# dojo-sim/Dojo.jl

Measured on NVIDIA H100. Metric: env-steps/sec (forward step!), higher is better.
Workload: dtype f64

## Files before the change

### dojo.jl_b200/csrc/dojo_b200.cu

```cuda
#include <cuda_runtime.h>

#include <algorithm>
#include <climits>
#include <cstdio>
#include <cstdlib>
#include <cstring>
#include <string>
#include <vector>

#include "../../include/dojo_b200.h"
#include "dojo_step_kernel.cuh"
#include "dojo_kin.cuh"
#include "dojo_kinjac.cuh"
#include "dojo_envs.cuh"
#include "dojo_storage.cuh"

using namespace dj;

extern "C" __attribute__((visibility("hidden"))) const void* dojo_cm_step_kernel(int grad);
static const void* step_kernel_fn(bool any_contact, bool grad, bool plan_smem, bool small = false) {
  if (any_contact) return dojo_cm_step_kernel(grad ? 1 : 0);
  if (plan_smem && !getenv("DOJO_B200_GENERIC_PLAN")) {
    if (!grad && small) return (const void*)dojo_step_kernel<false, true, false, true>;
    return grad ? (const void*)dojo_step_kernel<true, true> : (const void*)dojo_step_kernel<false, true>;
// ... 290 lines not shown

  Plan& P = h->plan;
  std::memset(&P, 0, sizeof(P));
  P.Nb = Nb; P.Ne = Ne; P.Ni = Ni; P.nres = nres; P.nu = nu; P.nz = 13 * Nb; P.nw = nw;
  P.h = d->timestep; P.input_scaling = d->input_scaling;
  std::memcpy(P.g, d->gravity, sizeof(P.g));
  int a = 0;
  P.sol_off = a; a += nres;
  P.rhs_off = a; a += nres;
  P.sav_off = a; a += nres;
  P.red_off = a; a += 4 * nw + 2;
  for (int b = 0; b < Nb; ++b) { bodies[b].st_off = a; a += 7; }
  for (int b = 0; b < Nb; ++b) { bodies[b].cst_off = a; a += 6; }
  for (int j = 0; j < Ne; ++j) {
    JointDev& J = joints[j];
    const int slot_len = (J.flags & JF_FULL) ? kSlotC : kSlot;
    J.slot_c = a; a += slot_len;
    if (J.parent >= 0) { J.slot_p = a; a += slot_len; } else J.slot_p = -1;
    J.Lc_off = a; a += 6 * joint_nq(J);
    if (J.parent >= 0) { J.Gp_off = a; a += 6 * joint_nq(J); } else J.Gp_off = -1;
    J.lim_off = a; a += ((J.flags & JF_FULL) ? 2 * kLim : kLim) * J.nb2_r;
  }
  for (int c = 0; c < Ni; ++c) {
    ContactDev& C = contacts[c];
    C.slot = a; a += kSlotC;
    C.J_off = a; a += 6 * (C.tn >> 8);
    C.G_off = a; a += 6 * (C.tn >> 8);
    C.rec_off = a; a += 3;
  }
  P.mat_off = a;
  for (int j = 0; j < Ne; ++j) { if (joints[j].parent >= 0) { joints[j].S_off = a; a += kScratch; } else joints[j].S_off = -1; }
  for (int b = 0; b < Nb; ++b) { bodies[b].D_off = a; a += 36; }
  for (int j = 0; j < Ne; ++j) {
    JointDev& J = joints[j];
    const int nq = joint_nq(J);
    J.D_off = a; a += nq * nq;
    J.Uc_off = a; a += 6 * nq;
    if (J.parent >= 0) {
      J.Up_off = a; a += 6 * nq;
      J.Lp_off = a; a += 6 * nq;
      const bool bb_full = (J.flags & JF_FULL) != 0;
      if (J.damper_r != 0.0 || J.nb2_r > 0 || (J.flags & JF_TRA_DAMPER)) { J.BBpc_off = a; a += bb_full ? 36 : 18; J.BBcp_off = a; a += bb_full ? 36 : 9; } else { J.BBpc_off = J.BBcp_off = -1; }
    } else { J.Up_off = J.Lp_off = J.BBpc_off = J.BBcp_off = -1; }
  }
  P.mat_len = a - P.mat_off;
  P.arena_len = a;
  {
    const int first_slot = Ne > 0 ? joints[0].slot_c : P.mat_off;
    const int span = P.mat_off - first_slot;
    const int per_pass = (nw == 4) ? 32 : 16;
    P.ls_pair = ((nw == 2 || nw == 4) && Nb <= per_pass && Ne <= per_pass && Ni <= per_pass && span + nres <= P.mat_len && !getenv("DOJO_B200_NO_LS_PAIR")) ? 1 : 0;
    P.jpair = (!h->any_contact && !getenv("DOJO_B200_NO_JOINT_PAIR")) ? 1 : 0;
    P.ls_assist = getenv("DOJO_B200_NO_LS_ASSIST") ? 0 : 1;
    P.ls_slot_delta = span;
    P.ls_res2_off = P.mat_off + span;
  }
  h->arena_bytes = (size_t)((a + 1) & ~1) * sizeof(double);

  std::vector<int> ucol;
  {
    int r = 0;
    for (int j = 0; j < Ne; ++j) { joints[j].r_off = r; r += joint_nq(joints[j]); }
    for (int b = 0; b < Nb; ++b) { bodies[b].r_off = r; r += 6; }
    P.n_red = r;
    P.ncol = 12 * Nb + nu;
    for (int j = 0; j < Ne; ++j)
      for (int k = 0; k < joints[j].nfree_t + joints[j].nfree_r; ++k) { ucol.push_back(j); ucol.push_back(k); }
    for (int pass = 0; pass < 4 && (32 >> pass) >= nw; ++pass) {
      P.ch = 32 >> pass;
      int g = P.arena_len;
      for (int b = 0; b < Nb; ++b) { bodies[b].gb_off = g; g += 30; }
      for (int c = 0; c < Ni; ++c) { contacts[c].gc_off = g; g += 36; }
      for (int j = 0; j < Ne; ++j) {
        JointDev& J = joints[j];
        J.gj_off = g; g += 12 * joint_nq(J) + 144 + 12 * (J.nfree_t + J.nfree_r);
        if (J.parent >= 0) { J.gv_off = g; g += 6 * P.ch; } else J.gv_off = -1;
      }
      P.gvec_off = g; g += P.n_red * P.ch;
      P.grad_len = g;
      if ((size_t)g * sizeof(double) <= 113 * 1024) break;
      if (pass >= 1 && (size_t)P.arena_len * sizeof(double) > 100 * 1024 && (size_t)g * sizeof(double) <= 225 * 1024) break;
    }
    h->grad_bytes = (size_t)((P.grad_len + 1) & ~1) * sizeof(double);
  }

  std::vector<int> ilist;
  for (int b = 0; b < Nb; ++b) {
    bodies[b].g_off = (int)ilist.size();
    for (int c = 0; c < Ni; ++c) if (contacts[c].body == b) ilist.push_back(contacts[c].slot);
    bodies[b].g_ncontact = (int)ilist.size() - bodies[b].g_off;
    auto slot_entry = [&](const JointDev& J, int slot) { return (J.flags & JF_FULL) ? (slot | (1 << 30)) : slot; };
    ilist.push_back(slot_entry(joints[parent_joint[b]], joints[parent_joint[b]].slot_c));
    for (int j = 0; j < Ne; ++j) if (joints[j].parent == b) ilist.push_back(slot_entry(joints[j], joints[j].slot_p));
    bodies[b].g_cnt = (int)ilist.size() - bodies[b].g_off;
  }

  for (int b = 0; b < Nb; ++b) {
    bodies[b].pjoint = parent_joint[b];
    bodies[b].cj_off = (int)ilist.size();
    for (int j = 0; j < Ne; ++j) if (joints[j].parent == b) ilist.push_back(j);
    bodies[b].cj_cnt = (int)ilist.size() - bodies[b].cj_off;
    bodies[b].ct_off = (int)ilist.size();
    for (int c = 0; c < Ni; ++c) if (contacts[c].body == b) ilist.push_back(c);
    bodies[b].ct_cnt = (int)ilist.size() - bodies[b].ct_off;
  }

// ... 1494 lines not shown
```

### dojo.jl_b200/csrc/dojo_grad.cuh

```cuda
#pragma once
#include "dojo_kernels.cuh"

namespace dj {

DJ_DEV void st_block33(double* B, int ld, int r0, int c0, const M33& m, double sgn = 1.0) {
#pragma unroll
  for (int i = 0; i < 3; ++i)
#pragma unroll
    for (int j = 0; j < 3; ++j) B[(r0 + i) * ld + c0 + j] = sgn * m.m[i][j];
}
DJ_DEV void add_block33(double* B, int ld, int r0, int c0, const M33& m, double sgn = 1.0) {
#pragma unroll
  for (int i = 0; i < 3; ++i)
#pragma unroll
    for (int j = 0; j < 3; ++j) B[(r0 + i) * ld + c0 + j] += sgn * m.m[i][j];
}
DJ_DEV M33 transport(V3 w, double h) { return transpose(rotmat(qmap(w, h))); }

DJ_DEV void grad_body(Ctx& c, int idx) {
  const Plan& P = *c.P;
  double* A = c.A;
  const BodyDev& bd = c.bodies[idx];
  double* rec = A + bd.gb_off;
  V3 w15 = ld3(rec + 27);
// ... 552 lines not shown
            if (k < st.n) acc += Dc[r * st.n + k] * t[k];
          V[(st.r_off + r) * ch + lane] = acc;
        }
      }
    }
    __syncwarp();
  }
}

DJ_DEV void grad_write_column(Ctx& c, const double* V, int ch, int col, int lane, int b0, int bstride, double* __restrict__ Fz, double* __restrict__ Fu,
                              double* __restrict__ Fc) {
  const Plan& P = *c.P;
  const double* A = c.A;
  const int ng = 12 * P.Nb;
  double* out = col < ng ? Fz + (size_t)col * ng : (col < P.ncol ? Fu + (size_t)(col - ng) * ng : Fc + (size_t)(col - P.ncol) * ng);
  for (int b = b0; b < P.Nb; b += bstride) {
    const BodyDev& bd = c.bodies[b];
    const double* rec = A + bd.gb_off;
    V3 dv = v3(V[(bd.r_off + 0) * ch + lane], V[(bd.r_off + 1) * ch + lane], V[(bd.r_off + 2) * ch + lane]);
    V3 dw = v3(V[(bd.r_off + 3) * ch + lane], V[(bd.r_off + 4) * ch + lane], V[(bd.r_off + 5) * ch + lane]);
    V3 dx = P.h * dv;
    V3 dphi = ldm33(rec + 18) * dw;
    if (col < ng && col / 12 == b) {
      const int k = col - 12 * b;
      if (k < 3) { if (k == 0) dx.x += 1.0; else if (k == 1) dx.y += 1.0; else dx.z += 1.0; }
      else if (k >= 6 && k < 9) {
        const double* M = rec + 9;
        dphi.x += M[0 * 3 + (k - 6)]; dphi.y += M[1 * 3 + (k - 6)]; dphi.z += M[2 * 3 + (k - 6)];
      }
    }
    double* o = out + 12 * b;
    o[0] = dx.x; o[1] = dx.y; o[2] = dx.z;
    o[3] = dv.x; o[4] = dv.y; o[5] = dv.z;
    o[6] = dphi.x; o[7] = dphi.y; o[8] = dphi.z;
    o[9] = dw.x; o[10] = dw.y; o[11] = dw.z;
  }
}

DJ_DEV bool gradients(Ctx& c, double* __restrict__ Fz, double* __restrict__ Fu, double* __restrict__ Fc) {
  const Plan& P = *c.P;
  double* A = c.A;
  const WarpRole& role = c.roles[c.warp];
  for (int p = 0; p < role.npass; ++p) {
    const int idx = role_item(role, p, c.lane);
    if (idx < 0) continue;
    if (role.type[p] == ROLE_BODY) grad_body(c, idx);
    else if (role.type[p] == ROLE_CONTACT) grad_contact(c, idx);
    else grad_joint(c, idx);
  }
  for (int j = c.tid; j < P.Ne; j += c.nthreads)
    if (c.joints[j].gv_off >= 0)
      for (int t = 0; t < 6 * P.ch; ++t) A[c.joints[j].gv_off + t] = 0.0;
  slot_sync(c);
  bool ok = factorize(c);
  const int chw = P.ch / P.nw;
  double* V = A + P.gvec_off + c.warp * P.n_red * chw;
  const int gvo = c.warp * 6 * chw;
  const int parts = 32 / chw, part = c.lane / chw, l = c.lane - part * chw;
  const int ncol = P.ncol + (Fc ? 5 * P.Ni : 0);
  for (int c0 = c.warp * chw; c0 < ncol; c0 += P.ch) {
    if (part == 0 && c0 + l < ncol) grad_build_rhs(c, V, chw, c0 + l, l);
    __syncwarp();
    grad_solve_columns(c, V, chw, gvo, c0, ncol);
    if (c0 + l < ncol) grad_write_column(c, V, chw, c0 + l, l, part, parts, Fz, Fu, Fc);
    __syncwarp();
  }
  slot_sync(c);
  return ok;
}

}
```

### dojo.jl_b200/csrc/dojo_kernels.cuh

```cuda
#pragma once
#include "dojo_linalg.cuh"
#include "dojo_plan.h"

namespace dj {

#ifdef DJ_ANY_CONTACT
#define DJ_SLOT_OFF(raw) ((raw) & 0x3fffffff)
#define DJ_SLOT_FULL(raw) (((raw) >> 30) & 1)
#else
#define DJ_SLOT_OFF(raw) (raw)
#endif
#ifdef DJ_ANY_CONTACT
DJ_DEV int contact_type(const ContactDev& cd) { return cd.tn & 0xff; }
DJ_DEV int contact_nh(const ContactDev& cd) { return cd.tn >> 8; }
#endif

DJ_DEV V3 ld3(const double* p) { return V3{p[0], p[1], p[2]}; }
DJ_DEV void st3(double* p, V3 v) { p[0] = v.x; p[1] = v.y; p[2] = v.z; }
DJ_DEV void add3(double* p, V3 v) { p[0] += v.x; p[1] += v.y; p[2] += v.z; }
DJ_DEV M33 ldm33(const double* p) {
  M33 r;
#pragma unroll
  for (int i = 0; i < 3; ++i)
#pragma unroll
    for (int j = 0; j < 3; ++j) r.m[i][j] = p[3 * i + j];
  return r;
}
DJ_DEV void stm33(double* p, const M33& a) {
#pragma unroll
  for (int i = 0; i < 3; ++i)
#pragma unroll
    for (int j = 0; j < 3; ++j) p[3 * i + j] = a.m[i][j];
}
DJ_DEV Quat ldq(const double* p) { return Quat{p[0], p[1], p[2], p[3]}; }

struct Ctx {
  double* A;
  const Plan* P;
  const BodyDev* bodies;
  const JointDev* joints;
  const ContactDev* contacts;
  const ElimStep* steps;
  const int* sched;
  const int* ilist;
  const WarpRole* roles;
  const int* ucol;
  int tid, nthreads, warp, lane;
  int sd;
  int bar;
  double mu;
  int slot, nslots, slot_stride;
  double* arena0;
  int* s_int;
  double* s_dbl;
  int apar, assist;
#ifdef DJ_PROFILE
  long long t_eval_jac, t_eval_ls, t_fact, t_solve, t_misc, t_align, t_cone, t_center, t_rolewait, t_last;
  long long f_fold, f_inv, f_rm, f_schur, f_bar, f_last;
#endif
};
#ifdef DJ_PROFILE
#define DJ_TICK(c, field) { long long _t = clock64(); (c).field += _t - (c).t_last; (c).t_last = _t; }
#define DJ_FTICK(c, field) { long long _t = clock64(); (c).field += _t - (c).f_last; (c).f_last = _t; }
#else
#define DJ_TICK(c, field) {}
#define DJ_FTICK(c, field) {}
#endif

#ifdef DJ_HOSTEMU
DJ_DEV void slot_sync(const Ctx& c) { hostemu_bar_sync(c.bar, c.nthreads); }
#else
DJ_DEV void slot_sync(const Ctx& c) { asm volatile("bar.sync %0, %1;" ::"r"(c.bar), "r"(c.nthreads) : "memory"); }
#endif

constexpr int kMaxAssistTrials = 16;
struct AlignInfo { int n_live, owner; };
#ifdef DJ_HOSTEMU
DJ_DEV void cta_barrier() { __syncthreads(); }
#else
__device__ __noinline__ void cta_barrier() { __syncthreads(); }
#endif
DJ_DEV AlignInfo cta_align(Ctx& c, bool live) {
  int* fl = c.s_int + 8 + 8 * c.apar;
  c.apar ^= 1;
  if (c.tid == 0) fl[c.slot] = live ? 1 : 0;
  cta_barrier();
  AlignInfo r;
  r.n_live = 0; r.owner = -1;
  for (int q = 0; q < c.nslots; ++q)
    if (fl[q]) { r.n_live++; r.owner = q; }
  return r;
}
DJ_DEV void assist_release(Ctx& c) {
  if (!c.assist) return;
  if (c.tid == 0) c.s_int[24] = 0;
  cta_barrier();
  c.assist = 0;
}

template <bool SMALL>
DJ_DEV int slot_warps(const Ctx& c) { return SMALL ? 2 : c.P->nw; }

template <bool SMALL = false>
DJ_DEV void block_nanmax2(const Ctx& c, double& a, double& b) {
  double* red = c.A + c.P->red_off;
  a = warp_nanmax(a);
  b = warp_nanmax(b);
  if (slot_warps<SMALL>(c) == 1) return;
  if (c.lane == 0) { red[2 * c.warp] = a; red[2 * c.warp + 1] = b; }
  slot_sync(c);
  a = red[0]; b = red[1];
// ... 1001 lines not shown
  const Plan& P = *c.P;
  double* A = c.A;
  const WarpRole& role = c.roles[c.warp];
  const bool pl = SMALL || P.ls_pair != 0;
  const int half = pl ? (c.lane >> 4) : 0;
  const int ln = pl ? (c.lane & 15) : c.lane;
  const bool on = (half == 0) || pair;
  const double f = half ? 0.5 * fk : fk;
  double* res = W + (half ? P.ls_res2_off : P.sav_off);
  c.sd = (int)(W - A) + (half ? P.ls_slot_delta : 0);
  double rv = 0.0, bv = 0.0;
  for (int p = 0; p < role.npass; ++p) {
    const int idx = on ? role_item(role, p, ln) : -1;
    if (idx < 0) continue;
    if (role.type[p] == ROLE_BODY) eval_body<false>(c, idx, f, res);
    else if (role.type[p] == ROLE_CONTACT) eval_contact<false>(c, idx, f, res, rv, bv);
    else eval_joint<false>(c, idx, f, res, rv, bv);
  }
  slot_sync(c);
  for (int p = 0; p < role.npass; ++p) {
    const int idx = on ? role_item(role, p, ln) : -1;
    if (idx < 0 || role.type[p] != ROLE_BODY) continue;
    const BodyDev& bd = c.bodies[idx];
    double* rb = res + bd.sol_off;
    for (int g = 0; g < bd.g_cnt; ++g) {
      const double* s = A + DJ_SLOT_OFF(c.ilist[bd.g_off + g]) + c.sd;
      add3(rb, ld3(s));
      add3(rb + 3, ld3(s + 3));
    }
#pragma unroll
    for (int i = 0; i < 6; ++i) rv = nanmax(rv, fabs(rb[i]));
  }
  c.sd = 0;
#pragma unroll
  for (int o = 8; o > 0; o >>= 1) {
    rv = nanmax(rv, __shfl_xor_sync(0xffffffffu, rv, o));
    bv = nanmax(bv, __shfl_xor_sync(0xffffffffu, bv, o));
  }
  if (!pl) {
    rv = nanmax(rv, __shfl_xor_sync(0xffffffffu, rv, 16));
    bv = nanmax(bv, __shfl_xor_sync(0xffffffffu, bv, 16));
  }
  double* red = W + P.red_off;
  if ((c.lane & 15) == 0) { red[4 * c.warp + 2 * (c.lane >> 4)] = rv; red[4 * c.warp + 2 * (c.lane >> 4) + 1] = bv; }
  slot_sync(c);
  rvA = red[0]; bvA = red[1]; rvB = red[2]; bvB = red[3];
  for (int w = 1; w < slot_warps<SMALL>(c); ++w) {
    rvA = nanmax(rvA, red[4 * w]); bvA = nanmax(bvA, red[4 * w + 1]);
    rvB = nanmax(rvB, red[4 * w + 2]); bvB = nanmax(bvB, red[4 * w + 3]);
  }
  slot_sync(c);
}

template <bool SMALL = false>
DJ_DEV bool factorize(Ctx& c) {
  const Plan& P = *c.P;
  double* A = c.A;
  bool ok = true;
  const int half = c.lane >> 4, l = c.lane & 15;
  const unsigned mask = 0xffffu << (16 * half);
#ifdef DJ_PROFILE
  c.f_last = clock64();
#endif
  for (int ph = 0; ph < P.nphase; ++ph) {
    const int s0 = c.sched[2 * (ph * slot_warps<SMALL>(c) + c.warp)], sn = c.sched[2 * (ph * slot_warps<SMALL>(c) + c.warp) + 1];
    for (int s = s0 + half; s < s0 + sn; s += 2) {
      const ElimStep& st = c.steps[s];
      double* Dc = A + st.d_off;
      if (st.fold_cnt > 0) {
        for (int t = l; t < st.n * st.n; t += 16) {
          double acc = Dc[t];
          for (int k = 0; k < st.fold_cnt; ++k) acc += A[c.ilist[st.fold_off + k] + t];
          Dc[t] = acc;
        }
        __syncwarp(mask);
      }
      DJ_FTICK(c, f_fold)
      ok = block_inverse(Dc, st.n, st.n, l, mask) && ok;
      DJ_FTICK(c, f_inv)
      for (int i = 0; i < st.nnb; ++i) right_multiply_inplace(A + st.nb[i].L_off, Dc, st.nb[i].n, st.n, l, mask);
      DJ_FTICK(c, f_rm)
      for (int i = 0; i < st.nnb; ++i)
        for (int j = 0; j < st.nnb; ++j)
          schur_update(A + st.tgt[i][j], st.nb[j].ld, A + st.nb[i].L_off + st.nb[j].U_row, st.n, A + st.nb[j].U_off, st.nb[i].n, st.nb[j].U_k,
                       st.nb[j].n, l, mask);
      DJ_FTICK(c, f_schur)
    }
    slot_sync(c);
    DJ_FTICK(c, f_bar)
  }
  int* flag = (int*)(A + P.red_off);
  const bool wok = __all_sync(0xffffffffu, ok);
  if (c.lane == 0) flag[c.warp] = wok ? 1 : 0;
  slot_sync(c);
  bool all = true;
  for (int w = 0; w < slot_warps<SMALL>(c); ++w) all = all && (flag[w] != 0);
  slot_sync(c);
  return all;
}

DJ_DEV double dot6(const double* a, const double* b, int n) {
  double e = 0.0, o = 0.0;
#pragma unroll
  for (int k = 0; k < 6; k += 2) {
    if (k < n) e = fma(a[k], b[k], e);
    if (k + 1 < n) o = fma(a[k + 1], b[k + 1], o);
  }
  return e + o;
}

template <bool SMALL = false>
DJ_DEV void solve(Ctx& c, int vec_off) {
  const Plan& P = *c.P;
  double* A = c.A;
  double* x = A + vec_off;
  const int lane = c.lane;
  const int half = lane >> 4, l = lane & 15;
  const int sub = l >> 3, li = l & 7;
  const WarpRole& role = c.roles[c.warp];
  for (int p = 0; p < role.npass; ++p) {
    const int idx = role_item(role, p, lane);
    if (idx < 0) continue;
    if (role.type[p] == ROLE_CONTACT) condense_contact(c, idx, x);
    else if (role.type[p] == ROLE_JOINT) condense_joint(c, idx, x);
  }
  slot_sync(c);
  for (int p = 0; p < role.npass; ++p) {
    const int idx = role_item(role, p, lane);
    if (idx < 0 || role.type[p] != ROLE_BODY) continue;
    const BodyDev& bd = c.bodies[idx];
    double* xb = x + bd.sol_off;
    for (int g = 0; g < bd.g_cnt; ++g) {
      const double* s = A + DJ_SLOT_OFF(c.ilist[bd.g_off + g]);
      add3(xb, ld3(s));
      add3(xb + 3, ld3(s + 3));
    }
  }
  slot_sync(c);
  for (int ph = 0; ph < P.nphase; ++ph) {
    const int s0 = c.sched[2 * (ph * slot_warps<SMALL>(c) + c.warp)], sn = c.sched[2 * (ph * slot_warps<SMALL>(c) + c.warp) + 1];
    for (int it = 0; 2 * it < sn; ++it) {
      const bool act = 2 * it + half < sn;
      const ElimStep& st = c.steps[s0 + 2 * it + (act ? half : 0)];
      double* xc = x + st.vec_off;
      if (act && st.fold_cnt > 0 && l < st.n) {
        double acc = xc[l];
        for (int k = 0; k < st.fold_cnt; ++k) {
          double* v = A + c.ilist[st.fold_off + k] + 36;
          acc += v[l];
          v[l] = 0.0;
        }
        xc[l] = acc;
      }
      __syncwarp();
      if (act && sub < st.nnb && li < st.nb[sub].n) {
        const ElimNb& nb = st.nb[sub];
        const double* L = A + nb.L_off + li * st.n;
        const double acc = dot6(L, xc, st.n);
        double* tgt = nb.fwd_abs >= 0 ? A + nb.fwd_abs : x + nb.vec_off;
        tgt[li] -= acc;
      }
      __syncwarp();
    }
    slot_sync(c);
  }
  for (int ph = P.nphase - 1; ph >= 0; --ph) {
    const int s0 = c.sched[2 * (ph * slot_warps<SMALL>(c) + c.warp)], sn = c.sched[2 * (ph * slot_warps<SMALL>(c) + c.warp) + 1];
    for (int it = (sn + 1) / 2 - 1; it >= 0; --it) {
      const bool act = 2 * it + half < sn;
      const ElimStep& st = c.steps[s0 + 2 * it + (act ? half : 0)];
      const double* Dc = A + st.d_off;
      double* xc = x + st.vec_off;
      if (act && st.nnb > 0 && l < st.n) {
        double acc = 0.0;
        for (int j = 0; j < st.nnb; ++j) {
          const ElimNb& nb = st.nb[j];
          int r = l - nb.U_row;
          if (r >= 0 && r < nb.U_k) {
            acc += dot6(A + nb.U_off + r * nb.n, x + nb.vec_off, nb.n);
          }
        }
        xc[l] -= acc;
      }
      __syncwarp();
      double acc = 0.0;
      if (act && l < st.n) acc = dot6(Dc + l * st.n, xc, st.n);
      __syncwarp();
      if (act && l < st.n) xc[l] = acc;
      __syncwarp();
    }
    slot_sync(c);
  }
  for (int p = 0; p < role.npass; ++p) {
    const int idx = role_item(role, p, lane);
    if (idx < 0) continue;
    if (role.type[p] == ROLE_CONTACT) recover_contact(c, idx, x);
    else if (role.type[p] == ROLE_JOINT) recover_joint(c, idx, x);
  }
  slot_sync(c);
}

DJ_DEV double ort_step(double lam, double dl, double tau) { return dl < 0.0 ? fmin(1.0, -tau * lam / dl) : 1.0; }
DJ_DEV double soc_step(double l0, double l1, double l2, double d0, double d1, double d2, double tau) {
  const double eps = 1e-14;
  double ll = fmax(l0 * l0 - (l1 * l1 + l2 * l2), 1e-25) + eps;
  double ld = l0 * d0 - (l1 * d1 + l2 * d2) + eps;
  double rs = ld / ll;
  double sq = sqrt(ll);
  double fct = (ld / sq + d0) / (l0 / sq + 1.0);
  double r1 = d1 / sq - fct * l1 / ll;
  double r2 = d2 / sq - fct * l2 / ll;
  double nr = sqrt(r1 * r1 + r2 * r2);
  return (nr - rs > 0.0) ? fmin(1.0, tau / (nr - rs)) : 1.0;
}
template <bool SMALL = false>
DJ_DEV double cone_line_search(Ctx& c, double tau_ort, double tau_soc) {
  const Plan& P = *c.P;
  const double* sol = c.A + P.sol_off;
  const double* dl = c.A + P.rhs_off;
  const WarpRole& role = c.roles[c.warp];
  double a = 1.0;
  for (int p = 0; p < role.npass; ++p) {
#ifndef DJ_ANY_CONTACT
    if (role.type[p] == ROLE_CONTACT && role.count[p] <= 16) {
      const int ci = c.lane >> 1;
      if (ci < role.count[p]) {
        const ContactDev& cd = c.contacts[role.first[p] + ci];
        const int o = cd.sol_off + 4 * (c.lane & 1);
        const double* v = sol + o;
        const double* dv = dl + o;
        a = fmin(a, ort_step(v[0], dv[0], tau_ort));
        a = fmin(a, soc_step(v[1], v[2], v[3], dv[1], dv[2], dv[3], tau_soc));
      }
      continue;
    }
#endif
    const int idx = role_item(role, p, c.lane);
    if (idx < 0) continue;
    if (role.type[p] == ROLE_CONTACT) {
      const ContactDev& cd = c.contacts[idx];
      const double* s = sol + cd.sol_off;
#ifdef DJ_ANY_CONTACT
      if (contact_type(cd) != 2) {
        const int n2 = 2 * contact_nh(cd);
        for (int i = 0; i < n2; ++i) a = fmin(a, ort_step(s[i], dl[cd.sol_off + i], tau_ort));
        continue;
      }
#endif
      const double* g = s + 4;
      const double* ds = dl + cd.sol_off;
      const double* dg = ds + 4;
      a = fmin(a, ort_step(s[0], ds[0], tau_ort));
// ... 140 lines not shown
    if (mode == 0) { DJ_TICK(c, t_eval_jac) } else { DJ_TICK(c, t_eval_ls) }
    if (mode == 1) {
      if (c.assist) {
        const int per = (SMALL || P.ls_pair != 0) ? 2 : 1;
        const int ntr = min(per * c.nslots, o.max_ls - ls_k);
        bool accepted = false;
        for (int j = 0; j < ntr; ++j) {
          rv = c.s_dbl[2 + 2 * ls_k]; bv = c.s_dbl[3 + 2 * ls_k];
          if ((rv > rvio) && (bv > bvio) && (ls_k + 1 < o.max_ls)) { fk *= 0.5; ls_k += 1; continue; }
          accepted = true;
          break;
        }
        if (!accepted) continue;
        assist_release(c);
      } else if ((rv > rvio) && (bv > bvio) && (ls_k + 1 < o.max_ls)) {
        fk *= 0.5; ls_k += 1;
        if (!pair) continue;
        rv = rv2; bv = bv2;
        if ((rv > rvio) && (bv > bvio) && (ls_k + 1 < o.max_ls)) { fk *= 0.5; ls_k += 1; continue; }
      }
      fsel = fk;
      bool made = (!(rv < o.rtol) && (rv < 0.8 * rvio)) || (!(bv < o.btol) && (bv < 0.8 * bvio));
      no_progress = made ? max(no_progress - 1, 0) : no_progress + 1;
      rvio = rv; bvio = bv;
      if (no_progress >= o.no_progress_max) undercut *= o.no_progress_undercut;
      double* sol = A + P.sol_off;
      const double* dl = A + P.rhs_off;
      if (fsel != 0.0) {
        for (int t = c.tid; t < P.nres; t += c.nthreads) sol[t] += fsel * dl[t];
        slot_sync(c);
        if (c.tid < P.Nb) {
          double* w = sol + c.bodies[c.tid].sol_off + 3;
          double wmax = 3.9 / (P.h * P.h);
          double wd = w[0] * w[0] + w[1] * w[1] + w[2] * w[2];
          if (wd > wmax) { double k = wmax / wd; w[0] *= k; w[1] *= k; w[2] *= k; }
        }
        slot_sync(c);
      }
      if ((rvio != rvio) || (bvio != bvio)) { status = 3; break; }
      if (ndone >= o.max_iter) break;
      if (TRACE && c.tid == 0) { trace_row(trace, ndone, rvio, bvio, alpha_tr, mutarget, ls_k + 1); rows_tr = ndone + 1; }
      if ((rvio < o.rtol) && (bvio < o.btol)) { status = 0; break; }
      mode = 0; fk = 0.0;
      continue;
    }
    if (first) { rvio = rv; bvio = bv; first = false; }
    if (TRACE && c.tid == 0 && rows_tr == 0 && o.max_iter > 0) { trace_row(trace, 0, rvio, bvio, 1.0, 0.0, 0); rows_tr = 1; }
    if ((rvio != rvio) || (bvio != bvio)) { status = 3; assist_release(c); break; }
    if (ndone >= o.max_iter) { assist_release(c); break; }
    if ((rvio < o.rtol) && (bvio < o.btol)) { status = 0; assist_release(c); break; }
    ndone += 1;
    for (int t = c.tid; t < P.nres; t += c.nthreads) A[P.sav_off + t] = A[P.rhs_off + t];
    slot_sync(c);
    DJ_TICK(c, t_misc)
    if (!factorize<SMALL>(c)) { status = 3; assist_release(c); break; }
    DJ_TICK(c, t_fact)
    double alpha = 1.0;
    for (int pass = 0; pass < 2; ++pass) {
      DJ_TICK(c, t_misc)
      solve<SMALL>(c, P.rhs_off);
      DJ_TICK(c, t_solve)
      double mx = fmax(rvio, bvio);
      double tau = (pass == 0) ? 0.95 : fmax(0.95, 1.0 - mx * mx);
      DJ_TICK(c, t_misc)
      alpha = cone_line_search<SMALL>(c, tau, fmin(tau, 0.95));
      DJ_TICK(c, t_cone)
      if (pass == 0) {
        double nu, nuaff;
        centering<SMALL>(c, alpha, nu, nuaff);
        double ratio = nuaff / (nu + 1e-20);
        double sig = (ratio != ratio) ? ratio : fmin(fmax(ratio, 0.0), 1.0);
        sig = sig * sig * sig;
        double sn = sig * nu;
        mutarget = (sn != sn) ? sn : fmax(sn, o.btol / undercut);
        c.mu = mutarget;
        correction(c);
        for (int t = c.tid; t < P.nres; t += c.nthreads) A[P.rhs_off + t] = A[P.sav_off + t];
        slot_sync(c);
        DJ_TICK(c, t_center)
      }
    }
    mode = 1; fk = alpha; ls_k = 0;
    if (TRACE) alpha_tr = alpha;
  }
  if (TRACE && c.tid == 0)
    for (int k = rows_tr * 5; k < o.max_iter * 5; ++k) trace[k] = nan("");
  *iters = ndone;
  return status;
}

template <bool SMALL = false>
DJ_DEV void ls_assist_loop(Ctx& c, const Options& o, int owner, int rank) {
  const Plan& P = *c.P;
  double* own = c.A;
  const int per = (SMALL || P.ls_pair != 0) ? 2 : 1;
  for (;;) {
    cta_barrier();
    if (c.s_int[24] == 0) break;
    const int k0 = c.s_int[25] + per * rank;
    if (k0 < o.max_ls) {
      double f = c.s_dbl[0];
      for (int q = 0; q < per * rank; ++q) f *= 0.5;
      c.mu = c.s_dbl[1];
      const bool pair = (per == 2) && (k0 + 1 < o.max_ls);
      double rv, bv, rv2, bv2;
      c.A = c.arena0 + (size_t)owner * c.slot_stride;
      evaluate_ls<SMALL>(c, own, f, pair, rv, bv, rv2, bv2);
      c.A = own;
      if (c.tid == 0) {
        c.s_dbl[2 + 2 * k0] = rv; c.s_dbl[3 + 2 * k0] = bv;
        if (pair) { c.s_dbl[4 + 2 * k0] = rv2; c.s_dbl[5 + 2 * k0] = bv2; }
      }
    }
    cta_barrier();
  }
  c.mu = 0.0;
}

}
```

### dojo.jl_b200/csrc/dojo_plan.h

```cpp
#pragma once
#include <stdint.h>

namespace dj {

constexpr double kReg = 1.0e-10;
constexpr int kSlot = 15;
constexpr int kSlotC = 42;
constexpr int kScratch = 42;
constexpr int kLim = 12;

enum RoleType { ROLE_BODY = 0, ROLE_CONTACT = 1, ROLE_JOINT = 2 };

struct BodyDev {
  double mass;
  double J[9];
  int sol_off;
  int st_off;
  int cst_off;
  int D_off;
  int g_off, g_cnt, g_ncontact;
  int pjoint;
  int cj_off, cj_cnt;
  int ct_off, ct_cnt;
  int r_off;
// ... 32 lines not shown
#if defined(__CUDACC__) || defined(DJ_HOSTEMU)
#define DJ_PLAN_FN __host__ __device__ inline
#else
#define DJ_PLAN_FN inline
#endif
DJ_PLAN_FN int joint_nq(const JointDev& j) { return j.ne + j.nb2_r; }
DJ_PLAN_FN const double* joint_tra_params(const JointDev& j) { return j.Ct + 3 * j.nl_t; }
DJ_PLAN_FN double* joint_tra_params(JointDev& j) { return j.Ct + 3 * j.nl_t; }

struct ContactDev {
  int body, sol_off;
  double mu, radius;
  double n[3], t[6], o[3], off[3];
  int J_off, G_off, rec_off;
  int slot;
  int gc_off;
  int tn;
};
static_assert(sizeof(ContactDev) == 168, "ContactDev layout is part of the kernels' addressing");

struct ElimNb {
  int n, vec_off;
  int r_off;
  int gv_off;
  int fwd_abs;
  int L_off;
  int U_off, U_k;
  int U_row;
  int ld;
  int row0;
};
struct ElimStep {
  int d_off, n, vec_off;
  int r_off;
  int gfold_off;
  int nnb;
  ElimNb nb[2];
  int tgt[2][2];
  int fold_off, fold_cnt;
};

struct WarpRole {
  int npass;
  int type[3], first[3], count[3];
};

struct Plan {
  int Nb, Ne, Ni, nres, nu, nz;
  int nw;
  int nphase;
  int ls_pair, ls_slot_delta, ls_res2_off;
  int ls_assist;
  int jpair;
  double h, input_scaling, g[3];
  int sol_off, rhs_off, sav_off, red_off, mat_off, mat_len, arena_len;
  const BodyDev* bodies;
  const JointDev* joints;
  const ContactDev* contacts;
  const ElimStep* steps;
  const int* sched;
  const int* ilist;
  const WarpRole* roles;
  int n_red;
  int ncol;
  int ch;
  int gvec_off;
  int grad_len;
  const int* ucol;
};

struct Options {
  double rtol, btol, undercut, no_progress_undercut;
  int max_iter, max_ls, no_progress_max;
};

}
```

### dojo.jl_b200/csrc/dojo_step_kernel.cuh

```cuda
#pragma once
#include "../../include/dojo_b200.h"
#include "dojo_grad.cuh"

namespace dj {

struct StepArgs {
  Plan plan;
  Options opts;
  int B;
  const double* Z;
  const double* U;
  const double* Fext;
  double* Zn;
  double* sol;
  int32_t* status;
  int32_t* iters;
  int* done_count;
  int* done_list;
  double* sol_raw;
  double* Fz;
  double* Fu;
  double* Fc;
  uint32_t flags;
  int* counter;
// ... 57 lines not shown
  c.warp = c.tid >> 5;
  c.lane = c.tid & 31;
  c.bar = 1 + slot;
  c.sd = 0;
  c.mu = 0.0;
  c.slot = slot; c.nslots = blockDim.x / slot_threads; c.slot_stride = a.slot_stride; c.arena0 = arena;
  c.s_int = s_env; c.s_dbl = reinterpret_cast<double*>(s_env + 32);
  c.apar = 0; c.assist = 0;
  {
    const char* gb = a.plan_blob;
    const char* sb = nullptr;
    if (PLAN_SMEM || a.plan_smem_off >= 0) {
      int4* dst = reinterpret_cast<int4*>(arena + a.plan_smem_off);
      const int4* src = reinterpret_cast<const int4*>(a.plan_blob);
#ifndef DJ_HOSTEMU
      __shared__ __align__(8) unsigned long long s_plan_bar;
      const unsigned bar = (unsigned)__cvta_generic_to_shared(&s_plan_bar);
      if (threadIdx.x == 0) {
        asm volatile("mbarrier.init.shared::cta.b64 [%0], 1;" ::"r"(bar) : "memory");
        asm volatile("fence.proxy.async.shared::cta;" ::: "memory");
      }
      __syncthreads();
      if (threadIdx.x == 0) {
        const unsigned bytes = (unsigned)a.plan_smem_bytes;
        asm volatile("mbarrier.arrive.expect_tx.shared::cta.b64 _, [%0], %1;" ::"r"(bar), "r"(bytes) : "memory");
        asm volatile("cp.async.bulk.shared::cluster.global.mbarrier::complete_tx::bytes [%0], [%1], %2, [%3];"
                     ::"r"((unsigned)__cvta_generic_to_shared(dst)), "l"(src), "r"(bytes), "r"(bar) : "memory");
      }
      {
        unsigned done = 0;
        while (!done)
          asm volatile("{ .reg .pred p; mbarrier.try_wait.parity.shared::cta.b64 p, [%1], 0; selp.u32 %0, 1, 0, p; }" : "=r"(done) : "r"(bar) : "memory");
      }
#else
      for (int i = threadIdx.x; i < a.plan_smem_bytes / 16; i += blockDim.x) dst[i] = src[i];
      __syncthreads();
#endif
      sb = reinterpret_cast<const char*>(dst);
    }
#define DJ_TABLE(k) ((PLAN_SMEM || (sb && ((a.plan_smem_mask >> (k)) & 1))) ? sb + a.plan_off[k] : gb + a.plan_off[k])
    c.bodies = reinterpret_cast<const BodyDev*>(DJ_TABLE(0));
    c.joints = reinterpret_cast<const JointDev*>(DJ_TABLE(1));
    c.contacts = reinterpret_cast<const ContactDev*>(DJ_TABLE(2));
    c.steps = reinterpret_cast<const ElimStep*>(DJ_TABLE(3));
    c.sched = reinterpret_cast<const int*>(DJ_TABLE(4));
    c.ilist = reinterpret_cast<const int*>(DJ_TABLE(5));
    c.roles = reinterpret_cast<const WarpRole*>(DJ_TABLE(6));
    c.ucol = reinterpret_cast<const int*>(DJ_TABLE(7));
#undef DJ_TABLE
  }
#ifdef DJ_PROFILE
  c.t_eval_jac = c.t_eval_ls = c.t_fact = c.t_solve = c.t_misc = c.t_align = c.t_cone = c.t_center = c.t_rolewait = 0; c.t_last = clock64();
  c.f_fold = c.f_inv = c.f_rm = c.f_schur = c.f_bar = 0;
  long long k_c0 = clock64(); unsigned long long k_t0; asm volatile("mov.u64 %0, %%globaltimer;" : "=l"(k_t0));
  int k_envs = 0;
  if (c.tid == 0 && a.prof) atomicMin(a.prof + 31, k_t0);
#endif
  if (!GRAD) asm volatile("griddepcontrol.launch_dependents;" ::: "memory");
  const Plan& P = a.plan;
  for (;;) {
    if (c.tid == 0) {
      int q = atomicAdd(a.counter, 1);
      int env = (q < a.B && a.order) ? a.order[q] : q;
      if (GRAD && a.done_list && q < a.B) {
        while ((env = ((volatile int*)a.done_list)[q]) < 0) __nanosleep(256);
        __threadfence();
      }
      s_env[slot] = env;
    }
    slot_sync(c);
    const int e = s_env[slot];
    slot_sync(c);
    if (e >= a.B) break;
    DJ_TICK(c, t_misc)
#ifdef DJ_PROFILE
    k_envs++;
    unsigned long long e_t0; asm volatile("mov.u64 %0, %%globaltimer;" : "=l"(e_t0));
#endif
    const double* z = a.Z + (size_t)e * P.nz;
    int worst = 0, iters = 0, status = 0;
    if (!GRAD) {
      for (int t = 0; t < a.T; ++t) {
        const double* u = a.U ? a.U + ((size_t)t * a.B + e) * P.nu : nullptr;
        const double* fx = a.Fext ? a.Fext + (size_t)e * 6 * P.Nb : nullptr;
        prologue(c, z, u, fx, false);
        status = mehrotra<TRACE, SMALL>(c, a.opts, &iters, TRACE ? a.trace + (size_t)e * max(a.opts.max_iter, 0) * 5 : nullptr);
        worst = max(worst, status);
        double* zo = (a.traj ? a.traj + ((size_t)t * a.B + e) * P.nz : a.Zn + (size_t)e * P.nz);
        epilogue(c, zo, (a.flags & DOJO_FLAG_Q1_LITERAL_RETURN) != 0, (t + 1 == a.T) ? a.n_peers : 0, a.peer_buf, a.gather_off + (long long)e * P.nz);
        if (REC) {
          const size_t p = (size_t)t * a.B + e;
          for (int k = c.tid; k < P.nres; k += c.nthreads) a.sol_raw[p * P.nres + k] = c.A[P.sol_off + k];
          if (c.tid == 0) {
            a.status[p] = status;
            if (a.iters) a.iters[p] = iters;
          }
          if (a.done_list) {
            __threadfence();
            slot_sync(c);
            if (c.tid == 0) {
              const int pos = atomicAdd(a.done_count, 1);
              __threadfence();
              ((volatile int*)a.done_list)[pos] = (int)p;
            }
          }
        }
// ... 43 lines not shown
        if (jd.flags & JF_LIM_TRA) {
          for (int i = 0; i < 2 * jd.nb_r; ++i) dst[i] = src[jd.ne + i];
          for (int i = 0; i < jd.ne; ++i) dst[2 * jd.nb_r + i] = src[i];
        } else
#endif
        {
        for (int i = 0; i < jd.nl_t; ++i) dst[i] = src[i];
        for (int i = 0; i < 2 * jd.nb_r; ++i) dst[jd.nl_t + i] = src[jd.ne + i];
        for (int i = 0; i < jd.nl_r; ++i) dst[jd.nl_t + 2 * jd.nb_r + i] = src[jd.nl_t + i];
        }
      }
    }
    if (c.tid == 0) {
      if (a.status && !REC) a.status[e] = status;
      if (!GRAD && !REC) {
        if (a.iters) a.iters[e] = iters;
        if (a.prev_iters) a.prev_iters[e] = iters;
      }
#ifdef DJ_PROFILE
      if (a.prof) { unsigned long long e_t1; asm volatile("mov.u64 %0, %%globaltimer;" : "=l"(e_t1)); a.prof[32 + 2 * e] = e_t0 - k_t0g(a.prof); a.prof[33 + 2 * e] = e_t1 - e_t0; }
#endif
    }
    if (!GRAD && !REC && a.done_list) {
      __threadfence();
      slot_sync(c);
      if (c.tid == 0) {
        const int pos = atomicAdd(a.done_count, 1);
        __threadfence();
        ((volatile int*)a.done_list)[pos] = e;
      }
    }
    slot_sync(c);
  }
  for (;;) {
    const AlignInfo ai = cta_align(c, false);
    if (ai.n_live == 0) break;
    if (!GRAD && P.ls_assist && ai.n_live == 1 && a.opts.max_ls <= kMaxAssistTrials) ls_assist_loop<SMALL>(c, a.opts, ai.owner, slot < ai.owner ? slot + 1 : slot);
  }
  if (!GRAD && a.n_peers > 0) {
    if (threadIdx.x == 0) {
      __threadfence_system();
      for (int r = 0; r < a.n_peers; ++r) atomicAdd_system(a.peer_flag[r], 1ull);
    }
  }
  if (GRAD) asm volatile("griddepcontrol.wait;" ::: "memory");
#ifdef DJ_PROFILE
  DJ_TICK(c, t_misc)
  if (c.lane == 0 && a.prof) atomicAdd(a.prof + 17 + c.warp, (unsigned long long)c.t_rolewait);
  if (c.tid == 0 && a.prof) {
    atomicAdd(a.prof + 0, (unsigned long long)c.t_eval_jac); atomicAdd(a.prof + 1, (unsigned long long)c.t_eval_ls);
    atomicAdd(a.prof + 2, (unsigned long long)c.t_fact); atomicAdd(a.prof + 3, (unsigned long long)c.t_solve); atomicAdd(a.prof + 4, (unsigned long long)c.t_misc);
    atomicAdd(a.prof + 5, (unsigned long long)c.f_fold); atomicAdd(a.prof + 6, (unsigned long long)c.f_inv); atomicAdd(a.prof + 7, (unsigned long long)c.f_rm);
    atomicAdd(a.prof + 8, (unsigned long long)c.f_schur); atomicAdd(a.prof + 9, (unsigned long long)c.f_bar);
    unsigned long long k_t1; asm volatile("mov.u64 %0, %%globaltimer;" : "=l"(k_t1));
    atomicMax(a.prof + 10, (unsigned long long)(clock64() - k_c0)); atomicMax(a.prof + 11, k_t1 - k_t0);
    atomicMax(a.prof + 12, (unsigned long long)k_envs); atomicAdd(a.prof + 13, (unsigned long long)(clock64() - k_c0));
    atomicAdd(a.prof + 14, (unsigned long long)c.t_align); atomicAdd(a.prof + 15, (unsigned long long)c.t_cone); atomicAdd(a.prof + 16, (unsigned long long)c.t_center);
  }
#endif
}


}
```

Baseline: 459,700.

## Fuse forward substitution of first solve pass into factorization

Splits solve into a condense_rhs step and a solve that can skip forward substitution. During the first interior-point pass, the forward elimination of the right-hand side is done inside factorize, folding child contributions and applying L blocks as each elimination step runs. This removes the separate forward phase loop and its per-phase block barriers. The fused path relies on plan fields (fwd_abs, vec_off) and zeroing of fold vectors, and it reorders factorize after condense_rhs. It also adds profiling counters and an env var to disable the fusion.

```diff
diff --git a/dojo.jl_b200/csrc/dojo_b200.cu b/dojo.jl_b200/csrc/dojo_b200.cu
--- a/dojo.jl_b200/csrc/dojo_b200.cu
+++ b/dojo.jl_b200/csrc/dojo_b200.cu
@@ -366,6 +366,7 @@
     P.ls_pair = ((nw == 2 || nw == 4) && Nb <= per_pass && Ne <= per_pass && Ni <= per_pass && span + nres <= P.mat_len && !getenv("DOJO_B200_NO_LS_PAIR")) ? 1 : 0;
     P.jpair = (!h->any_contact && !getenv("DOJO_B200_NO_JOINT_PAIR")) ? 1 : 0;
     P.ls_assist = getenv("DOJO_B200_NO_LS_ASSIST") ? 0 : 1;
+    P.fuse_fwd = getenv("DOJO_B200_NO_FUSED_FWD") ? 0 : 1;
     P.ls_slot_delta = span;
     P.ls_res2_off = P.mat_off + span;
   }
diff --git a/dojo.jl_b200/csrc/dojo_grad.cuh b/dojo.jl_b200/csrc/dojo_grad.cuh
--- a/dojo.jl_b200/csrc/dojo_grad.cuh
+++ b/dojo.jl_b200/csrc/dojo_grad.cuh
@@ -628,7 +628,7 @@
     if (c.joints[j].gv_off >= 0)
       for (int t = 0; t < 6 * P.ch; ++t) A[c.joints[j].gv_off + t] = 0.0;
   slot_sync(c);
-  bool ok = factorize(c);
+  bool ok = factorize(c, -1);
   const int chw = P.ch / P.nw;
   double* V = A + P.gvec_off + c.warp * P.n_red * chw;
   const int gvo = c.warp * 6 * chw;
diff --git a/dojo.jl_b200/csrc/dojo_kernels.cuh b/dojo.jl_b200/csrc/dojo_kernels.cuh
--- a/dojo.jl_b200/csrc/dojo_kernels.cuh
+++ b/dojo.jl_b200/csrc/dojo_kernels.cuh
@@ -57,6 +57,7 @@
 #ifdef DJ_PROFILE
   long long t_eval_jac, t_eval_ls, t_fact, t_solve, t_misc, t_align, t_cone, t_center, t_rolewait, t_last;
   long long f_fold, f_inv, f_rm, f_schur, f_bar, f_last;
+  long long s_fwd, s_bwd, s_bar, s_cr;
 #endif
 };
 #ifdef DJ_PROFILE
@@ -1164,13 +1165,25 @@
   slot_sync(c);
 }
 
+DJ_DEV double dot6(const double* a, const double* b, int n) {
+  double e = 0.0, o = 0.0;
+#pragma unroll
+  for (int k = 0; k < 6; k += 2) {
+    if (k < n) e = fma(a[k], b[k], e);
+    if (k + 1 < n) o = fma(a[k + 1], b[k + 1], o);
+  }
+  return e + o;
+}
+
 template <bool SMALL = false>
-DJ_DEV bool factorize(Ctx& c) {
+DJ_DEV bool factorize(Ctx& c, int fwd_off) {
   const Plan& P = *c.P;
   double* A = c.A;
   bool ok = true;
   const int half = c.lane >> 4, l = c.lane & 15;
+  const int sub = l >> 3, li = l & 7;
   const unsigned mask = 0xffffu << (16 * half);
+  double* x = fwd_off >= 0 ? A + fwd_off : nullptr;
 #ifdef DJ_PROFILE
   c.f_last = clock64();
 #endif
@@ -1185,6 +1198,16 @@
           for (int k = 0; k < st.fold_cnt; ++k) acc += A[c.ilist[st.fold_off + k] + t];
           Dc[t] = acc;
         }
+        if (x && l < st.n) {
+          double* xc = x + st.vec_off;
+          double acc = xc[l];
+          for (int k = 0; k < st.fold_cnt; ++k) {
+            double* v = A + c.ilist[st.fold_off + k] + 36;
+            acc += v[l];
+            v[l] = 0.0;
+          }
+          xc[l] = acc;
+        }
         __syncwarp(mask);
       }
       DJ_FTICK(c, f_fold)
@@ -1192,6 +1215,12 @@
       DJ_FTICK(c, f_inv)
       for (int i = 0; i < st.nnb; ++i) right_multiply_inplace(A + st.nb[i].L_off, Dc, st.nb[i].n, st.n, l, mask);
       DJ_FTICK(c, f_rm)
+      if (x && sub < st.nnb && li < st.nb[sub].n) {
+        const ElimNb& nb = st.nb[sub];
+        const double acc = dot6(A + nb.L_off + li * st.n, x + st.vec_off, st.n);
+        double* tgt = nb.fwd_abs >= 0 ? A + nb.fwd_abs : x + nb.vec_off;
+        tgt[li] -= acc;
+      }
       for (int i = 0; i < st.nnb; ++i)
         for (int j = 0; j < st.nnb; ++j)
           schur_update(A + st.tgt[i][j], st.nb[j].ld, A + st.nb[i].L_off + st.nb[j].U_row, st.n, A + st.nb[j].U_off, st.nb[i].n, st.nb[j].U_k,
@@ -1211,25 +1240,14 @@
   return all;
 }
 
-DJ_DEV double dot6(const double* a, const double* b, int n) {
-  double e = 0.0, o = 0.0;
-#pragma unroll
-  for (int k = 0; k < 6; k += 2) {
-    if (k < n) e = fma(a[k], b[k], e);
-    if (k + 1 < n) o = fma(a[k + 1], b[k + 1], o);
-  }
-  return e + o;
-}
-
-template <bool SMALL = false>
-DJ_DEV void solve(Ctx& c, int vec_off) {
-  const Plan& P = *c.P;
+DJ_DEV void condense_rhs(Ctx& c, int vec_off) {
   double* A = c.A;
   double* x = A + vec_off;
   const int lane = c.lane;
-  const int half = lane >> 4, l = lane & 15;
-  const int sub = l >> 3, li = l & 7;
   const WarpRole& role = c.roles[c.warp];
+#ifdef DJ_PROFILE
+  c.f_last = clock64();
+#endif
   for (int p = 0; p < role.npass; ++p) {
     const int idx = role_item(role, p, lane);
     if (idx < 0) continue;
@@ -1249,7 +1267,22 @@
     }
   }
   slot_sync(c);
-  for (int ph = 0; ph < P.nphase; ++ph) {
+  DJ_FTICK(c, s_cr)
+}
+
+template <bool SMALL = false>
+DJ_DEV void solve(Ctx& c, int vec_off, bool fwd) {
+  const Plan& P = *c.P;
+  double* A = c.A;
+  double* x = A + vec_off;
+  const int lane = c.lane;
+  const int half = lane >> 4, l = lane & 15;
+  const int sub = l >> 3, li = l & 7;
+  const WarpRole& role = c.roles[c.warp];
+#ifdef DJ_PROFILE
+  c.f_last = clock64();
+#endif
+  for (int ph = 0; fwd && ph < P.nphase; ++ph) {
     const int s0 = c.sched[2 * (ph * slot_warps<SMALL>(c) + c.warp)], sn = c.sched[2 * (ph * slot_warps<SMALL>(c) + c.warp) + 1];
     for (int it = 0; 2 * it < sn; ++it) {
       const bool act = 2 * it + half < sn;
@@ -1274,7 +1307,9 @@
       }
       __syncwarp();
     }
+    DJ_FTICK(c, s_fwd)
     slot_sync(c);
+    DJ_FTICK(c, s_bar)
   }
   for (int ph = P.nphase - 1; ph >= 0; --ph) {
     const int s0 = c.sched[2 * (ph * slot_warps<SMALL>(c) + c.warp)], sn = c.sched[2 * (ph * slot_warps<SMALL>(c) + c.warp) + 1];
@@ -1301,7 +1336,9 @@
       if (act && l < st.n) xc[l] = acc;
       __syncwarp();
     }
+    DJ_FTICK(c, s_bwd)
     slot_sync(c);
+    DJ_FTICK(c, s_bar)
   }
   for (int p = 0; p < role.npass; ++p) {
     const int idx = role_item(role, p, lane);
@@ -1310,6 +1347,7 @@
     else if (role.type[p] == ROLE_JOINT) recover_joint(c, idx, x);
   }
   slot_sync(c);
+  DJ_FTICK(c, s_cr)
 }
 
 DJ_DEV double ort_step(double lam, double dl, double tau) { return dl < 0.0 ? fmin(1.0, -tau * lam / dl) : 1.0; }
@@ -1556,13 +1594,18 @@
     ndone += 1;
     for (int t = c.tid; t < P.nres; t += c.nthreads) A[P.sav_off + t] = A[P.rhs_off + t];
     slot_sync(c);
-    DJ_TICK(c, t_misc)
-    if (!factorize<SMALL>(c)) { status = 3; assist_release(c); break; }
-    DJ_TICK(c, t_fact)
     double alpha = 1.0;
+    bool singular = false;
     for (int pass = 0; pass < 2; ++pass) {
       DJ_TICK(c, t_misc)
-      solve<SMALL>(c, P.rhs_off);
+      condense_rhs(c, P.rhs_off);
+      DJ_TICK(c, t_solve)
+      const bool fused = (pass == 0) && P.fuse_fwd;
+      if (pass == 0) {
+        if (!factorize<SMALL>(c, fused ? P.rhs_off : -1)) { singular = true; break; }
+        DJ_TICK(c, t_fact)
+      }
+      solve<SMALL>(c, P.rhs_off, !fused);
       DJ_TICK(c, t_solve)
       double mx = fmax(rvio, bvio);
       double tau = (pass == 0) ? 0.95 : fmax(0.95, 1.0 - mx * mx);
@@ -1584,6 +1627,7 @@
         DJ_TICK(c, t_center)
       }
     }
+    if (singular) { status = 3; assist_release(c); break; }
     mode = 1; fk = alpha; ls_k = 0;
     if (TRACE) alpha_tr = alpha;
   }
diff --git a/dojo.jl_b200/csrc/dojo_plan.h b/dojo.jl_b200/csrc/dojo_plan.h
--- a/dojo.jl_b200/csrc/dojo_plan.h
+++ b/dojo.jl_b200/csrc/dojo_plan.h
@@ -108,6 +108,7 @@
   int ls_pair, ls_slot_delta, ls_res2_off;
   int ls_assist;
   int jpair;
+  int fuse_fwd;
   double h, input_scaling, g[3];
   int sol_off, rhs_off, sav_off, red_off, mat_off, mat_len, arena_len;
   const BodyDev* bodies;
diff --git a/dojo.jl_b200/csrc/dojo_step_kernel.cuh b/dojo.jl_b200/csrc/dojo_step_kernel.cuh
--- a/dojo.jl_b200/csrc/dojo_step_kernel.cuh
+++ b/dojo.jl_b200/csrc/dojo_step_kernel.cuh
@@ -133,6 +133,7 @@
 #ifdef DJ_PROFILE
   c.t_eval_jac = c.t_eval_ls = c.t_fact = c.t_solve = c.t_misc = c.t_align = c.t_cone = c.t_center = c.t_rolewait = 0; c.t_last = clock64();
   c.f_fold = c.f_inv = c.f_rm = c.f_schur = c.f_bar = 0;
+  c.s_fwd = c.s_bwd = c.s_bar = c.s_cr = 0;
   long long k_c0 = clock64(); unsigned long long k_t0; asm volatile("mov.u64 %0, %%globaltimer;" : "=l"(k_t0));
   int k_envs = 0;
   if (c.tid == 0 && a.prof) atomicMin(a.prof + 31, k_t0);
@@ -282,6 +283,8 @@
     atomicAdd(a.prof + 2, (unsigned long long)c.t_fact); atomicAdd(a.prof + 3, (unsigned long long)c.t_solve); atomicAdd(a.prof + 4, (unsigned long long)c.t_misc);
     atomicAdd(a.prof + 5, (unsigned long long)c.f_fold); atomicAdd(a.prof + 6, (unsigned long long)c.f_inv); atomicAdd(a.prof + 7, (unsigned long long)c.f_rm);
     atomicAdd(a.prof + 8, (unsigned long long)c.f_schur); atomicAdd(a.prof + 9, (unsigned long long)c.f_bar);
+    atomicAdd(a.prof + 25, (unsigned long long)c.s_fwd); atomicAdd(a.prof + 26, (unsigned long long)c.s_bwd);
+    atomicAdd(a.prof + 27, (unsigned long long)c.s_bar); atomicAdd(a.prof + 28, (unsigned long long)c.s_cr);
     unsigned long long k_t1; asm volatile("mov.u64 %0, %%globaltimer;" : "=l"(k_t1));
     atomicMax(a.prof + 10, (unsigned long long)(clock64() - k_c0)); atomicMax(a.prof + 11, k_t1 - k_t0);
     atomicMax(a.prof + 12, (unsigned long long)k_envs); atomicAdd(a.prof + 13, (unsigned long long)(clock64() - k_c0));
```

New measurement: 461,100, median of 6. Within noise of the previous version (+0.3%).
